# ashual/scene_generation

Hardware: AMD Instinct MI355X
Metric: images/sec G+D step, 128x128 <=8-obj scene graphs (higher is better)
Workload: dtype f32

## Files before the change

### scene_generation_amd/csrc/common.h

```cpp
#pragma once
#include <hip/hip_runtime.h>
#include <stdint.h>
#include <stdio.h>
#include <atomic>
#include "../../include/sg2im_hip.h"

#define SG_WAVE 64

void sg_set_error(const char* fmt, ...);
int sg_check_indices_if_enabled(const int64_t* idx, int64_t n, int64_t lo, int64_t hi, const char* what, hipStream_t s);

#define SG_ARG_CHECK(cond, ...)                 \
  do {                                          \
    if (!(cond)) {                              \
      sg_set_error(__VA_ARGS__);                \
      return -1;                                \
    }                                           \
  } while (0)

#define SG_LAUNCH_CHECK(name)                                               \
  do {                                                                      \
    hipError_t e__ = hipGetLastError();                                     \
    if (e__ != hipSuccess) {                                                \
      sg_set_error("%s: launch failed: %s", name, hipGetErrorString(e__)); \
      return (int)e__;                                                      \
    }                                                                       \
  } while (0)

enum SgOpt {
  SG_OPT_TILE,
  SG_OPT_T128_MIN,
  SG_OPT_TILE3,
  SG_OPT_TILE3_MIN,
  SG_OPT_SPLIT_TARGET,
  SG_OPT_SPLIT_KMIN,
  SG_OPT_SPLITS,
  SG_OPT_FIXEDTAP,
  SG_OPT_WINO_WT,
  SG_OPT_W24_SMALL,
  SG_OPT_W24_S,
  SG_OPT_W24_PMIN,
  SG_OPT_WINO_ADJOINT,
  SG_OPT_WINO24,
  SG_OPT_LINEAR_NSUB,
  SG_OPT_LINEAR_SKINNY,
  SG_OPT_WGRAD_ROWSUM,
  SG_OPT_LAYOUT_REG,
  SG_OPT_LAYOUT_DSPLIT,
  SG_OPT_BN_BLOCKS,
  SG_OPT_INSTNORM_REG,
  SG_OPT_WGRAD_XCD,
  SG_OPT_WINO_REUSE,
  SG_OPT_WINO_FOLD_CELLS,
  SG_OPT_WINO_PIPE,
  SG_OPT_CHECK_INDICES,
  SG_OPT_LAST_BLOCK,
  SG_OPT_WINO_GEMM_TILE,
  SG_OPT_WINO43,
  SG_OPT_GCONV_FUSED_GATHER,
  SG_OPT_W24_GEMM_TILE,
  SG_OPT_WINO_IN_FUSE,
  SG_OPT_W43_NSUB,
  SG_OPT_W43_KFOLD,
  SG_OPT_WAVE_PRIO,
  SG_OPT_PAR_XCD_CHUNK,
  SG_OPT_W43_TAIL_SPLIT,
  SG_OPT_TAIL_SMAX,
  SG_OPT_TAIL_KTMIN,
  SG_OPT_W43_WGRAD_TILE,
  SG_OPT_PAR_SPLIT,
  SG_OPT_TAIL_CAPTURE,
  SG_OPT_WGRAD_PADDED,
  SG_OPT_COUNT
};
extern std::atomic<int> g_sg_opt[SG_OPT_COUNT];
static inline int sg_opt(int id) { return g_sg_opt[id].load(std::memory_order_relaxed); }
extern FILE* g_sg_launch_log;

enum {
  SG_K_IGEMM_BASE = 0, SG_K_IGEMM_COUNT = 48,
  SG_K_LINEAR = 48, SG_K_LAYOUT_FWD, SG_K_LAYOUT_BWD, SG_K_INSTNORM, SG_K_BATCHNORM, SG_K_ADAM, SG_K_SEGSUM,
  SG_K_CROP, SG_K_OTHER,
  SG_K_WINO_GEMM_128, SG_K_WINO_GEMM_64, SG_K_WINO_XFORM,
  SG_K_HEAD,
  SG_K_INSTNORM_BWD,
  SG_K_WINO24_GEMM,
  SG_K_WINO43_GEMM,
  SG_K_LAYOUT_TEST_PLANES,
  SG_K_DEPROCESS,
  SG_K_LAYOUT_RGB,
  SG_K_KMEANS_ASSIGN, SG_K_KMEANS_UPDATE, SG_K_KMEANS_RELOCATE, SG_K_KMEANS_PP,
  SG_K_SCENEGRAPH_CENTERS, SG_K_SCENEGRAPH_DERIVE, SG_K_SCENEGRAPH_AGREE,
  SG_K_MAXPOOL3S2, SG_K_ADD_RELU, SG_K_BN_FOLD, SG_K_SGD, SG_K_CLASSIFY_STATS,
  SG_K_RECT_CONV_T64, SG_K_RECT_CONV_T32, SG_K_RECT_CONV_T64W, SG_K_RECT_REDUCE, SG_K_INCEPTION_POOL, SG_K_RESIZE_BILINEAR,
  SG_K_SOFTMAX_ROWS, SG_K_INCEPTION_SCORE,
  SG_K_FID_MOMENTS,
  SG_K_WIDE_CONV, SG_K_LPIPS_INPUT, SG_K_LPIPS_LAYER,
  SG_K_FEAT_POLY, SG_K_FEAT_MANIFOLD,
  SG_K_PIL_RESIZE,
  SG_K_FIDINF_GRAMS, SG_K_FIDINF_TERMS,
  SG_K_COUNT
};
static inline int sg_igemm_kind(int family, int KS, int tile) {
  const int k = KS == 1 ? 0 : (KS == 3 ? 1 : (KS == 4 ? 2 : 3));
  return SG_K_IGEMM_BASE + family * 16 + k * 4 + tile;
}
extern int g_sg_prof_on;
void sg_prof_begin(int kind, hipStream_t s);
void sg_prof_end(int kind, hipStream_t s, double flops, double bytes);

struct SgProfScope {
  int kind; hipStream_t s; double flops, bytes; bool on;
  SgProfScope(int k, hipStream_t st, double f, double b) : kind(k), s(st), flops(f), bytes(b), on(g_sg_prof_on != 0) {
    if (on) sg_prof_begin(kind, s);
  }
  ~SgProfScope() { if (on) sg_prof_end(kind, s, flops, bytes); }
};

struct FastDiv {
  unsigned m, s, d;
  FastDiv() : m(0), s(0), d(1) {}
  explicit FastDiv(unsigned dd) : m(0), s(0), d(dd) {
    if (dd > 1) {
      unsigned sh = 0;
      while ((1u << sh) < dd) ++sh;
      m = (unsigned)((((uint64_t)1) << (31 + sh)) / dd + 1);
      s = sh - 1;
    }
  }
  __device__ __forceinline__ unsigned div(unsigned n) const { return d == 1 ? n : (__umulhi(n, m) >> s); }
};

static inline int sg_cdiv(int64_t a, int64_t b) { return (int)((a + b - 1) / b); }

__device__ __forceinline__ float sg_apply_act(float v, int act, float slope) {
  switch (act) {
    case SG_ACT_RELU: return v > 0.f ? v : 0.f;
    case SG_ACT_LEAKY: return v > 0.f ? v : v * slope;
    case SG_ACT_TANH: return tanhf(v);
    case SG_ACT_SIGMOID: return 1.f / (1.f + expf(-v));
    default: return v;
  }
}

__device__ __forceinline__ float sg_wave_sum(float v) {
#pragma unroll
  for (int o = 32; o > 0; o >>= 1) v += __shfl_xor(v, o, 64);
  return v;
}

__device__ __forceinline__ float sg_sum_strided(const float* __restrict__ p, size_t stride, int S) {
  float v = 0.f;
  for (int z0 = 0; z0 < S; z0 += 8) {
    float t[8];
#pragma unroll
    for (int e = 0; e < 8; ++e) t[e] = z0 + e < S ? p[(size_t)(z0 + e) * stride] : 0.f;
#pragma unroll
    for (int e = 0; e < 8; ++e)
      if (z0 + e < S) v += t[e];
  }
  return v;
}

__device__ __forceinline__ void sg_publish(float* p, float v) { __hip_atomic_store(p, v, __ATOMIC_RELAXED, __HIP_MEMORY_SCOPE_AGENT); }
__device__ __forceinline__ float sg_consume(const float* p) {
  return __hip_atomic_load(const_cast<float*>(p), __ATOMIC_RELAXED, __HIP_MEMORY_SCOPE_AGENT);
}
__device__ __forceinline__ bool sg_arrive_last(int* counter, int narrive, int* flag) {
  asm volatile("s_waitcnt vmcnt(0)" ::: "memory");
  __syncthreads();
  if (threadIdx.x == 0 && threadIdx.y == 0 && threadIdx.z == 0) {
    const int t = __hip_atomic_fetch_add(counter, 1, __ATOMIC_RELAXED, __HIP_MEMORY_SCOPE_AGENT);
    const int last = t == narrive - 1;
    if (last) __hip_atomic_store(counter, 0, __ATOMIC_RELAXED, __HIP_MEMORY_SCOPE_AGENT);
    *flag = last;
  }
  __syncthreads();
  return *flag != 0;
}
int* sg_counter_alloc(hipStream_t s, int n = 1, bool always = false, int family = 1);
float* sg_tail_scratch(hipStream_t s, size_t bytes);

__device__ __forceinline__ float sg_block_sum(float v, float* red) {
  const int lane = threadIdx.x & 63, wid = threadIdx.x >> 6, nw = (blockDim.x + 63) >> 6;
  v = sg_wave_sum(v);
  __syncthreads();
  if (lane == 0) red[wid] = v;
  __syncthreads();
  float t = 0.f;
  for (int i = 0; i < nw; ++i) t += red[i];
  return t;
}
```

### scene_generation_amd/csrc/igemm.hip

```cpp
#include "igemm_core.h"

namespace sgk {
thread_local double t_alg_bytes = 0.0;
std::mutex g_tab_mu;
std::map<TabKey, TabEntry> g_tabs;
size_t g_tab_bytes = 0;
}

namespace {
int check_desc(const sgConvDesc* d, const char* who) {
  SG_ARG_CHECK(d != nullptr, "%s: null desc", who);
  SG_ARG_CHECK(d->KS == 1 || d->KS == 3 || d->KS == 4 || d->KS == 7, "%s: kernel size %d unsupported", who, d->KS);
  SG_ARG_CHECK(d->stride == 1 || d->stride == 2, "%s: stride %d unsupported", who, d->stride);
  SG_ARG_CHECK(d->upsample == 1 || d->upsample == 2, "%s: upsample %d unsupported", who, d->upsample);
  SG_ARG_CHECK(d->N > 0 && d->C1 > 0 && d->C2 >= 0 && d->Cout > 0 && d->H > 0 && d->W > 0 && d->OH > 0 && d->OW > 0,
               "%s: non-positive dimension", who);
  SG_ARG_CHECK(!d->pad_reflect || d->pad < d->H * d->upsample, "%s: reflect pad too large", who);
  const double lim = SG_MAX_ELEMS;
  SG_ARG_CHECK((double)d->N * (d->C1 + d->C2) * d->H * d->W <= lim && (double)d->N * d->Cout * d->OH * d->OW <= lim &&
                   (double)d->N * (d->C1 + d->C2) * (d->H * d->upsample + 2.0 * d->pad) *
                           (d->W * d->upsample + 2.0 * d->pad) <= lim &&
                   (double)d->Cout * (d->C1 + d->C2) * d->KS * d->KS <= lim,
               "%s: a tensor has more than %.0f elements (32-bit offsets%s)", who, lim,
               SG_BUFLOAD ? ", buffer-load range masking" : "");
// ... 1119 lines not shown
      if (rb >= 0 && ca >= 0) v += acc[rb * PW + ca];
      if (rb >= 0 && cb >= 0) v += acc[rb * PW + cb];
      so[a * W + b] = v;
    }
  }
  __syncthreads();
  float* dstg = gx + ((size_t)n * C + c0) * HW;
  for (int i = threadIdx.x * 4; i < 64 * HW; i += 1024) {
    const int ch = i / HW, px = i - ch * HW;
    const float* sp = stage + ch * (HW + 1) + px;
    *reinterpret_cast<float4*>(dstg + i) = make_float4(sp[0], sp[1], sp[2], sp[3]);
  }
}

template <int TPT>
__global__ void __launch_bounds__(256) w43_output_in_kernel(const float* __restrict__ Mx, const float* __restrict__ bias,
                                                           const float* __restrict__ skip, float* __restrict__ ypre,
                                                           float* __restrict__ out, float* __restrict__ mean_o,
                                                           float* __restrict__ rstd_o, int N, int M, int H, int W, float eps, int act,
                                                           float slope) {
  extern __shared__ __attribute__((aligned(16))) float lds[];
  const int HW = H * W, TH = H / 4, TW = W / 4, NT = TH * TW, pitch = HW + 1;
  const int n = blockIdx.y, c0 = blockIdx.x * 64, c = threadIdx.x & 63, g = threadIdx.x >> 6, m = c0 + c;
  float* sa = lds;
  float* sb = lds + 64 * pitch;
  float* red = lds + 128 * pitch;
  const float b = bias ? bias[m] : 0.f;
  const size_t ld = (size_t)36 * M;
  float o[TPT][4][4];
  float s = 0.f;
#pragma unroll
  for (int k = 0; k < TPT; ++k) {
    const int t = g + 4 * k;
    if (t < NT) {
      const float* src = Mx + ((size_t)n * NT + t) * ld + m;
      float q[6][6];
#pragma unroll
      for (int i = 0; i < 36; ++i) q[i / 6][i % 6] = src[(size_t)i * M];
      w43_output_xform(q, o[k]);
#pragma unroll
      for (int a = 0; a < 4; ++a)
#pragma unroll
        for (int e = 0; e < 4; ++e) { o[k][a][e] += b; s += o[k][a][e]; }
    }
  }
  red[g * 64 + c] = s;
  __syncthreads();
  const float mean = (((red[c] + red[64 + c]) + red[128 + c]) + red[192 + c]) / (float)HW;
  __syncthreads();
  float qv = 0.f;
#pragma unroll
  for (int k = 0; k < TPT; ++k)
    if (g + 4 * k < NT) {
#pragma unroll
      for (int a = 0; a < 4; ++a)
#pragma unroll
        for (int e = 0; e < 4; ++e) { const float dlt = o[k][a][e] - mean; qv += dlt * dlt; }
    }
  red[g * 64 + c] = qv;
  __syncthreads();
  const float rstd = 1.f / sqrtf((((red[c] + red[64 + c]) + red[128 + c]) + red[192 + c]) / (float)HW + eps);
  if (g == 0) { mean_o[(size_t)n * M + m] = mean; rstd_o[(size_t)n * M + m] = rstd; }
#pragma unroll
  for (int k = 0; k < TPT; ++k) {
    const int t = g + 4 * k;
    if (t < NT) {
      const int ti = t / TW, tj = t - ti * TW;
#pragma unroll
      for (int a = 0; a < 4; ++a)
#pragma unroll
        for (int e = 0; e < 4; ++e) {
          const int px = (4 * ti + a) * W + 4 * tj + e;
          sa[c * pitch + px] = o[k][a][e];
          sb[c * pitch + px] = sg_apply_act((o[k][a][e] - mean) * rstd, act, slope);
        }
    }
  }
  __syncthreads();
  const size_t base = ((size_t)n * M + c0) * HW;
  for (int i = threadIdx.x * 4; i < 64 * HW; i += 1024) {
    const int ch = i / HW, px = i - ch * HW;
    const float* pa = sa + ch * pitch + px;
    const float* pb = sb + ch * pitch + px;
    *reinterpret_cast<float4*>(ypre + base + i) = make_float4(pa[0], pa[1], pa[2], pa[3]);
    float4 v = make_float4(pb[0], pb[1], pb[2], pb[3]);
    if (skip) {
      const float4 k4 = *reinterpret_cast<const float4*>(skip + base + i);
      v.x += k4.x; v.y += k4.y; v.z += k4.z; v.w += k4.w;
    }
    *reinterpret_cast<float4*>(out + base + i) = v;
  }
}

__global__ void __launch_bounds__(256) w43_gy_in_kernel(const float* __restrict__ gout, const float* __restrict__ ypre,
                                                       const float* __restrict__ mean_i, const float* __restrict__ rstd_i,
                                                       float* __restrict__ gconv, float* __restrict__ Ytp, float* __restrict__ gb_part,
                                                       int N, int M, int H, int W, int act, float slope) {
  extern __shared__ __attribute__((aligned(16))) float lds[];
  const int HW = H * W, pitch = HW + 1, TH = H / 4, TW = W / 4, NT = TH * TW;
  const int n = blockIdx.y, c0 = blockIdx.x * 64, tid = threadIdx.x, c = tid & 63, g = tid >> 6;
  float* pg = lds;
  float* px = lds + 64 * pitch;
  float* red = lds + 128 * pitch;
  const size_t base = ((size_t)n * M + c0) * HW;
  w43_stage_planes(gout + base, pg, HW, tid);
  w43_stage_planes(ypre + base, px, HW, tid);
  __syncthreads();
  const float mean = mean_i[(size_t)n * M + c0 + c], rstd = rstd_i[(size_t)n * M + c0 + c];
  float* gc = pg + c * pitch;
  const float* xc = px + c * pitch;
  float s1 = 0.f, s2 = 0.f;
  for (int t = g; t < NT; t += 4) {
    const int ti = t / TW, tj = t - ti * TW;
#pragma unroll
    for (int a = 0; a < 4; ++a)
#pragma unroll
      for (int e = 0; e < 4; ++e) {
        const int p = (4 * ti + a) * W + 4 * tj + e;
        const float z = (xc[p] - mean) * rstd;
        const float gp = gc[p] * act_grad_from_pre_w(z, act, slope);
        s1 += gp; s2 += gp * z;
      }
  }
  red[g * 64 + c] = s1;
  red[256 + g * 64 + c] = s2;
  __syncthreads();
  const float inv = 1.f / (float)HW;
  const float m1 = (((red[c] + red[64 + c]) + red[128 + c]) + red[192 + c]) * inv;
  const float m2 = (((red[256 + c] + red[320 + c]) + red[384 + c]) + red[448 + c]) * inv;
  const size_t P = (size_t)N * NT;
  float sb = 0.f;
  for (int t = g; t < NT; t += 4) {
    const int ti = t / TW, tj = t - ti * TW;
    float gt[4][4];
#pragma unroll
    for (int a = 0; a < 4; ++a)
#pragma unroll
      for (int e = 0; e < 4; ++e) {
        const int p = (4 * ti + a) * W + 4 * tj + e;
        const float z = (xc[p] - mean) * rstd;
        const float gp = gc[p] * act_grad_from_pre_w(z, act, slope);
        gt[a][e] = rstd * (gp - m1 - z * m2);
        gc[p] = gt[a][e];
        sb += gt[a][e];
      }
    float yt[6][6];
    w43_gy_xform(gt, yt);
    const size_t p = (size_t)n * NT + t;
#pragma unroll
    for (int i = 0; i < 6; ++i)
#pragma unroll
      for (int j = 0; j < 6; ++j) Ytp[((size_t)(i * 6 + j) * P + p) * M + c0 + c] = yt[i][j];
  }
  red[512 + g * 64 + c] = sb;
  __syncthreads();
  if (gb_part != nullptr && g == 0)
    gb_part[(size_t)n * M + c0 + c] = ((red[512 + c] + red[576 + c]) + red[640 + c]) + red[704 + c];
  for (int i = tid * 4; i < 64 * HW; i += 1024) {
    const int ch = i / HW, q = i - ch * HW;
    const float* sp = pg + ch * pitch + q;
    *reinterpret_cast<float4*>(gconv + base + i) = make_float4(sp[0], sp[1], sp[2], sp[3]);
  }
}

__global__ void w43_bias_sum_kernel(const float* __restrict__ part, float* __restrict__ gb, int N, int M) {
  const int m = blockIdx.x * blockDim.x + threadIdx.x;
  if (m >= M) return;
  float v = 0.f;
  for (int n0 = 0; n0 < N; n0 += 8) {
    float t[8];
#pragma unroll
    for (int e = 0; e < 8; ++e) t[e] = n0 + e < N ? part[(size_t)(n0 + e) * M + m] : 0.f;
#pragma unroll
    for (int e = 0; e < 8; ++e) v += t[e];
  }
  gb[m] = v;
}

__global__ void w43_wgrad_output_kernel(const float* __restrict__ T, float* __restrict__ gw, int M, int C) {
  const size_t idx = (size_t)blockIdx.x * blockDim.x + threadIdx.x;
  if (idx >= (size_t)M * C) return;
  const int c = (int)(idx % C);
  const size_t m = idx / C;
  const float* src = T + m * 36 * C + c;
  float q[6][6];
#pragma unroll
  for (int i = 0; i < 36; ++i) q[i / 6][i % 6] = src[(size_t)i * C];
  float o[3][3];
  w43_wgrad_xform(q, o);
  float* dst = gw + idx * 9;
#pragma unroll
  for (int a = 0; a < 3; ++a)
#pragma unroll
    for (int b = 0; b < 3; ++b) dst[a * 3 + b] = o[a][b];
}

void w43_launch_weight(const float* w, float* U, int R, int Cc, hipStream_t s) {
  SgProfScope xf(SG_K_WINO_XFORM, s, 0, 4.0 * 45.0 * (double)R * Cc);
  hipLaunchKernelGGL(w43_weight_kernel, dim3((R / 32) * (Cc / 32)), dim3(256), 0, s, w, U, R, Cc);
}
void w43_launch_input(const float* x, float* V, int N, int C, int H, int W, size_t P, hipStream_t s) {
  SgProfScope xf(SG_K_WINO_XFORM, s, 0, 4.0 * ((double)N * C * H * W + 36.0 * (double)P * C));
  const size_t lds = (size_t)64 * (H * W + 1) * sizeof(float);
  wino_lds_attr(&w43_input_kernel, lds);
  hipLaunchKernelGGL(w43_input_kernel, dim3(C / 64, N), dim3(256), lds, s, x, V, N, C, H, W);
}
void w43_launch_gy(const float* gy, float* Ytp, int N, int M, int H, int W, size_t P, hipStream_t s) {
  SgProfScope xf(SG_K_WINO_XFORM, s, 0, 4.0 * ((double)N * M * H * W + 36.0 * (double)P * M));
  const size_t lds = (size_t)64 * (H * W + 1) * sizeof(float);
  wino_lds_attr(&w43_gy_kernel, lds);
  hipLaunchKernelGGL(w43_gy_kernel, dim3(M / 64, N), dim3(256), lds, s, gy, Ytp, N, M, H, W);
}
void w43_launch_fold(const float* G, float* gx, int N, int C, int H, int W, size_t P, hipStream_t s) {
  SgProfScope xf(SG_K_WINO_XFORM, s, 0, 4.0 * (36.0 * (double)P * C + (double)N * C * H * W));
  const size_t lds = (size_t)64 * ((H + 2) * (W + 2) + 1 + H * W + 1) * sizeof(float);
  wino_lds_attr(&w43_fold_kernel, lds);
  hipLaunchKernelGGL(w43_fold_kernel, dim3(C / 64, N), dim3(256), lds, s, G, gx, N, C, H, W);
}
}

__device__ __forceinline__ void w24_bt(const float (&d)[5], float (&o)[5]) {
  o[0] = -2.f * d[0] - d[1] + 2.f * d[2] + d[3];
  o[1] = 2.f * d[1] + 3.f * d[2] + d[3];
  o[2] = -2.f * d[1] + d[2] + d[3];
  o[3] = d[3] - d[1];
  o[4] = -2.f * d[1] - d[2] + 2.f * d[3] + d[4];
}
__device__ __forceinline__ void w24_g(const float (&g)[4], float (&o)[5]) {
  o[0] = -0.5f * g[0];
  o[1] = (g[0] + g[1] + g[2] + g[3]) * (1.f / 6.f);
  o[2] = (g[0] - g[1] + g[2] - g[3]) * 0.5f;
  o[3] = (-g[0] + 2.f * g[1] - 4.f * g[2] + 8.f * g[3]) * (1.f / 6.f);
  o[4] = g[3];
}
__device__ __forceinline__ void w24_at(const float (&m)[5], float (&o)[2]) {
  o[0] = m[0] + m[1] + m[2] + m[3];
  o[1] = m[1] - m[2] - 2.f * m[3] + m[4];
}
__device__ __forceinline__ void w24_a(const float (&y)[2], float (&o)[5]) {
  o[0] = y[0]; o[1] = y[0] + y[1]; o[2] = y[0] - y[1]; o[3] = y[0] - 2.f * y[1]; o[4] = y[1];
}
__device__ __forceinline__ void w24_gt(const float (&t)[5], float (&o)[4]) {
  o[0] = -0.5f * t[0] + (t[1] - t[3]) * (1.f / 6.f) + 0.5f * t[2];
  o[1] = (t[1] + 2.f * t[3]) * (1.f / 6.f) - 0.5f * t[2];
  o[2] = (t[1] - 4.f * t[3]) * (1.f / 6.f) + 0.5f * t[2];
  o[3] = (t[1] + 8.f * t[3]) * (1.f / 6.f) - 0.5f * t[2] + t[4];
}

template <int KMAJ>
__global__ void w24_input_kernel(const float* __restrict__ x, float* __restrict__ V, int N, int C, int H, int W, int TH, int TW,
                                 int off, size_t Pstride, int Pc, int S) {
  const size_t P = (size_t)N * TH * TW, total = Pstride * C;
  const size_t idx = (size_t)blockIdx.x * blockDim.x + threadIdx.x;
  if (idx >= total) return;
  const size_t p = KMAJ ? idx % Pstride : idx / C;
  const int c = (int)(KMAJ ? idx / Pstride : idx % C);
  float d[5][5];
  if (p < P) {
    const int n = (int)(p / (TH * TW)), r = (int)(p - (size_t)n * TH * TW), ti = r / TW, tj = r - ti * TW;
    const float* xp = x + ((size_t)n * C + c) * H * W;
#pragma unroll
    for (int a = 0; a < 5; ++a) {
      const int ih = 2 * ti + off + a;
      const bool rok = (unsigned)ih < (unsigned)H;
#pragma unroll
      for (int b = 0; b < 5; ++b) {
        const int iw = 2 * tj + off + b;
        const bool ok = rok && (unsigned)iw < (unsigned)W;
        d[a][b] = ok ? xp[ih * W + iw] : 0.f;
      }
    }
  } else {
#pragma unroll
    for (int a = 0; a < 5; ++a)
#pragma unroll
      for (int b = 0; b < 5; ++b) d[a][b] = 0.f;
  }
  float t[5][5];
#pragma unroll
  for (int j = 0; j < 5; ++j) {
    const float col[5] = {d[0][j], d[1][j], d[2][j], d[3][j], d[4][j]};
    float o[5];
    w24_bt(col, o);
#pragma unroll
    for (int i = 0; i < 5; ++i) t[i][j] = o[i];
  }
#pragma unroll
  for (int i = 0; i < 5; ++i) {
    float o[5];
    w24_bt(t[i], o);
#pragma unroll
    for (int j = 0; j < 5; ++j) {
      const size_t xi = (size_t)(i * 5 + j);
      if (KMAJ) {
        const size_t sidx = p / (size_t)Pc, pc = p - sidx * (size_t)Pc;
        V[((xi * S + sidx) * C + c) * (size_t)Pc + pc] = o[j];
      } else {
        V[(xi * Pstride + p) * C + c] = o[j];
      }
    }
  }
}

__global__ void __launch_bounds__(256) w24_input_small_kernel(const float* __restrict__ x, float* __restrict__ V, int N, int C, int H,
                                                             int W, int TH, int TW, int off, size_t Pstride, int rows_per,
                                                             int pitch) {
  extern __shared__ __attribute__((aligned(16))) float pl[];
  const int HW = H * W;
  const int n = blockIdx.y, c0 = blockIdx.x * 64, tid = threadIdx.x;
  const int tr0 = (int)blockIdx.z * rows_per, tr1 = min(TH, tr0 + rows_per);
  const int lane = tid & 63, g = tid >> 6;
  const int rlo = max(0, 2 * tr0 + off), rhi = min(H, 2 * (tr1 - 1) + off + 5);
  {
    const int cnt = (rhi - rlo) * W;
    const float* src = x + ((size_t)n * C + c0) * HW + rlo * W;
    for (int ch = g; ch < 64; ch += 4)
      for (int e = lane; e < cnt; e += 64) pl[ch * pitch + e] = src[(size_t)ch * HW + e];
  }
  __syncthreads();
  const float* pc = pl + lane * pitch - rlo * W;
  const size_t P = (size_t)N * TH * TW;
  for (int t = tr0 * TW + g; t < tr1 * TW; t += 4) {
    const int ti = t / TW, tj = t - ti * TW;
    float d[5][5];
#pragma unroll
    for (int a = 0; a < 5; ++a) {
      const int ih = 2 * ti + off + a;
      const bool rok = (unsigned)ih < (unsigned)H;
#pragma unroll
      for (int b = 0; b < 5; ++b) {
        const int iw = 2 * tj + off + b;
        const bool ok = rok && (unsigned)iw < (unsigned)W;
        d[a][b] = ok ? pc[ih * W + iw] : 0.f;
      }
    }
    float tt[5][5];
#pragma unroll
    for (int j = 0; j < 5; ++j) {
      const float col[5] = {d[0][j], d[1][j], d[2][j], d[3][j], d[4][j]};
      float o[5];
      w24_bt(col, o);
#pragma unroll
      for (int i = 0; i < 5; ++i) tt[i][j] = o[i];
    }
    const size_t p = (size_t)n * TH * TW + t;
#pragma unroll
    for (int i = 0; i < 5; ++i) {
      float o[5];
      w24_bt(tt[i], o);
#pragma unroll
      for (int j = 0; j < 5; ++j) V[((size_t)(i * 5 + j) * Pstride + p) * C + c0 + lane] = o[j];
    }
  }
  if (n == 0 && blockIdx.z == 0)
    for (size_t p = P + g; p < Pstride; p += 4)
      for (int xi = 0; xi < 25; ++xi) V[((size_t)xi * Pstride + p) * C + c0 + lane] = 0.f;
}
inline bool w24_small_geom(int N, int C, int H, int W, int TH, int* rows_per_out, int* pitch_out) {
  int rows_per = (int)(((long)(C / 64) * N * TH + 2047) / 2048);
  if (rows_per < 1) rows_per = 1;
  const int nrows = std::min(H, 2 * rows_per + 3);
  const int pitch = (nrows * W) | 1;
  if ((size_t)64 * pitch * sizeof(float) > 64 * 1024) return false;
  *rows_per_out = rows_per;
  *pitch_out = pitch;
  return true;
}
void w24_input_pc(int kernel, const float* x, float* V, int N, int C, int H, int W, int TH, int TW, int off, size_t Pstride,
                  hipStream_t s) {
  const int HW = H * W;
  SgProfScope xf(SG_K_WINO_XFORM, s, 0, 4.0 * ((double)N * C * HW + 25.0 * (double)Pstride * C));
  if (kernel == SG_WK_IN_LDS) {
    int rows_per = 0, pitch = 0;
    w24_small_geom(N, C, H, W, TH, &rows_per, &pitch);
    const size_t lds = (size_t)64 * pitch * sizeof(float);
    wino_lds_attr(&w24_input_small_kernel, lds);
    hipLaunchKernelGGL(w24_input_small_kernel, dim3(C / 64, N, sg_cdiv(TH, rows_per)), dim3(256), lds, s, x, V, N, C, H, W, TH, TW, off,
                       Pstride, rows_per, pitch);
    return;
  }
  hipLaunchKernelGGL(w24_input_kernel<0>, dim3(sg_cdiv(Pstride * C, 256)), dim3(256), 0, s, x, V, N, C, H, W, TH, TW, off, Pstride, 0, 1);
}

__global__ void w24_weight_kernel(const float* __restrict__ w, float* __restrict__ U, int R, int Cc, int mode) {
  const size_t idx = (size_t)blockIdx.x * blockDim.x + threadIdx.x;
  if (idx >= (size_t)R * Cc) return;
  const int c = (int)(idx % Cc), r = (int)(idx / Cc);
  const float* g = w + (mode ? ((size_t)c * R + r) : ((size_t)r * Cc + c)) * 16;
  float k[4][4];
#pragma unroll
  for (int i = 0; i < 16; ++i) k[i >> 2][i & 3] = mode ? g[15 - i] : g[i];
  float t[5][4];
#pragma unroll
  for (int j = 0; j < 4; ++j) {
    const float col[4] = {k[0][j], k[1][j], k[2][j], k[3][j]};
    float o[5];
    w24_g(col, o);
#pragma unroll
    for (int i = 0; i < 5; ++i) t[i][j] = o[i];
  }
#pragma unroll
  for (int i = 0; i < 5; ++i) {
    float o[5];
    w24_g(t[i], o);
#pragma unroll
    for (int j = 0; j < 5; ++j) U[((size_t)(i * 5 + j) * R + r) * Cc + c] = o[j];
  }
}

__global__ void w24_output_kernel(const float* __restrict__ Mx, const float* __restrict__ bias, float* __restrict__ y, int N,
                                  int M, int OH, int OW, int TH, int TW, size_t Pstride, int act, float slope) {
  const size_t P = (size_t)N * TH * TW;
  const size_t idx = (size_t)blockIdx.x * blockDim.x + threadIdx.x;
  if (idx >= P * M) return;
  const size_t p = idx % P;
  const int m = (int)(idx / P);
  const float* src = Mx + (size_t)m * 25 * Pstride + p;
  float q[5][5];
#pragma unroll
  for (int i = 0; i < 25; ++i) q[i / 5][i % 5] = src[(size_t)i * Pstride];
  float sres[2][5];
#pragma unroll
  for (int j = 0; j < 5; ++j) {
    const float col[5] = {q[0][j], q[1][j], q[2][j], q[3][j], q[4][j]};
    float o[2];
    w24_at(col, o);
    sres[0][j] = o[0]; sres[1][j] = o[1];
  }
  const float b = bias ? bias[m] : 0.f;
  const int n = (int)(p / (TH * TW)), r = (int)(p - (size_t)n * TH * TW), ti = r / TW, tj = r - ti * TW;
  float* o = y + (((size_t)n * M + m) * OH + 2 * ti) * OW + 2 * tj;
#pragma unroll
  for (int a = 0; a < 2; ++a) {
    float v[2];
    w24_at(sres[a], v);
    if (2 * ti + a < OH) {
      o[a * OW] = sg_apply_act(v[0] + b, act, slope);
      if (2 * tj + 1 < OW) o[a * OW + 1] = sg_apply_act(v[1] + b, act, slope);
    }
  }
}

__global__ void w24_gy_kernel(const float* __restrict__ gy, float* __restrict__ Yt, int N, int M, int OH, int OW, int TH, int TW,
                              size_t Pstride, int Pc, int S) {
  const size_t P = (size_t)N * TH * TW;
  const size_t idx = (size_t)blockIdx.x * blockDim.x + threadIdx.x;
  if (idx >= Pstride * M) return;
  const size_t p = idx % Pstride;
  const int m = (int)(idx / Pstride);
  float y2[2][2] = {{0.f, 0.f}, {0.f, 0.f}};
  if (p < P) {
    const int n = (int)(p / (TH * TW)), r = (int)(p - (size_t)n * TH * TW), ti = r / TW, tj = r - ti * TW;
    const float* g = gy + (((size_t)n * M + m) * OH + 2 * ti) * OW + 2 * tj;
#pragma unroll
    for (int a = 0; a < 2; ++a)
#pragma unroll
      for (int b = 0; b < 2; ++b)
        if (2 * ti + a < OH && 2 * tj + b < OW) y2[a][b] = g[a * OW + b];
  }
  float t[5][2];
#pragma unroll
  for (int j = 0; j < 2; ++j) {
    const float col[2] = {y2[0][j], y2[1][j]};
    float o[5];
    w24_a(col, o);
#pragma unroll
    for (int i = 0; i < 5; ++i) t[i][j] = o[i];
  }
  const size_t sidx = p / (size_t)Pc, pc = p - sidx * (size_t)Pc;
#pragma unroll
  for (int i = 0; i < 5; ++i) {
    float o[5];
    w24_a(t[i], o);
#pragma unroll
    for (int j = 0; j < 5; ++j) Yt[(((size_t)(i * 5 + j) * S + sidx) * M + m) * (size_t)Pc + pc] = o[j];
  }
}

__global__ void w24_wgrad_output_kernel(const float* __restrict__ T, float* __restrict__ gw, int M, int C, int S) {
  const size_t idx = (size_t)blockIdx.x * blockDim.x + threadIdx.x;
  if (idx >= (size_t)M * C) return;
  const int c = (int)(idx % C), m = (int)(idx / C);
  const float* src = T + (size_t)m * 25 * S * C + c;
  float q[5][5];
#pragma unroll
  for (int i = 0; i < 25; ++i) q[i / 5][i % 5] = 0.f;
  for (int z = 0; z < S; ++z) {
    float t[25];
#pragma unroll
    for (int i = 0; i < 25; ++i) t[i] = src[((size_t)i * S + z) * C];
#pragma unroll
    for (int i = 0; i < 25; ++i) q[i / 5][i % 5] += t[i];
  }
  float t[4][5];
#pragma unroll
  for (int j = 0; j < 5; ++j) {
    const float col[5] = {q[0][j], q[1][j], q[2][j], q[3][j], q[4][j]};
    float o[4];
    w24_gt(col, o);
#pragma unroll
    for (int i = 0; i < 4; ++i) t[i][j] = o[i];
  }
  float* dst = gw + ((size_t)m * C + c) * 16;
#pragma unroll
  for (int i = 0; i < 4; ++i) {
    float o[4];
    w24_gt(t[i], o);
    *reinterpret_cast<float4*>(dst + i * 4) = make_float4(o[0], o[1], o[2], o[3]);
  }
}

struct W24Plan { int TH, TW, THd, TWd; size_t P, Ps, Pd, Pds; int S, Pc; };
bool w24_plan(const sgConvDesc* d, W24Plan* pl) {
  if (!d || d->KS != 4 || d->stride != 1 || d->C2 != 0 || d->upsample != 1 || d->pad_reflect || d->pad < 0 || d->pad > 3) return false;
  if (d->C1 % 128 != 0 || d->Cout % 128 != 0 || d->OH < 2 || d->OW < 2) return false;
  if (d->OH != d->H + 2 * d->pad - 3 || d->OW != d->W + 2 * d->pad - 3) return false;
  W24Plan p;
  p.TH = (d->OH + 1) / 2; p.TW = (d->OW + 1) / 2;
  p.THd = (d->H + 1) / 2; p.TWd = (d->W + 1) / 2;
  p.P = (size_t)d->N * p.TH * p.TW; p.Pd = (size_t)d->N * p.THd * p.TWd;
  p.Ps = (p.P + 127) / 128 * 128; p.Pds = (p.Pd + 127) / 128 * 128;
  const long t = 25L * (d->Cout / 128) * (d->C1 / 128);
  int S = (int)((400 + t - 1) / t);
  if (sg_opt(SG_OPT_W24_S) > 0) S = sg_opt(SG_OPT_W24_S);
  const int maxS = (int)(p.P / 256) > 0 ? (int)(p.P / 256) : 1;
  if (S > maxS) S = maxS;
  if (S < 1) S = 1;
  p.Pc = (int)(((p.P + S - 1) / S + 31) / 32 * 32);
  p.S = (int)((p.P + p.Pc - 1) / p.Pc);
  const double cm = d->C1 > d->Cout ? d->C1 : d->Cout;
  const double pm = (double)(p.Ps > p.Pds ? p.Ps : p.Pds) + 32.0 * p.S;
  if (!(25.0 * pm * cm < 2147483647.0 && 25.0 * (double)d->C1 * d->Cout < 2147483647.0)) return false;
  if (p.P < (size_t)sg_opt(SG_OPT_W24_PMIN)) return false;
  if (pl) *pl = p;
  return true;
}

int wino_class(const sgConvDesc* d) {
  if (!wino_ok(d)) return SG_WF_UNSUPPORTED;
  if (!(sg_opt(SG_OPT_WINO_ADJOINT) && d->pad_reflect && d->upsample == 1 && d->H * d->W <= 256 && (d->H * d->W) % 4 == 0 &&
        d->C1 % 64 == 0 && d->Cout % 64 == 0))
    return SG_WF_F23_GENERIC;
  if (!sg_opt(SG_OPT_WINO43) || d->H % 4 != 0 || d->W % 4 != 0) return SG_WF_F23_ADJOINT;
  const double P = (double)d->N * (d->H / 4) * (d->W / 4), Cmax = d->C1 > d->Cout ? d->C1 : d->Cout;
  return ((long)P % 64 == 0 && 36.0 * P * Cmax < SG_MAX_ELEMS && 36.0 * d->C1 * d->Cout < SG_MAX_ELEMS) ? SG_WF_F43 : SG_WF_F23_ADJOINT;
}
size_t wino_tiles(const sgConvDesc* d, int t) { return (size_t)d->N * (d->H * d->upsample / t) * (d->W * d->upsample / t); }
size_t wino_dgrad_tiles(const sgConvDesc* d) {
  const size_t T = (size_t)wino_tile(d);
  const size_t P = d->pad_reflect ? (size_t)d->N * (d->H * d->upsample / 2 + 1) * (d->W * d->upsample / 2 + 1) : wino_tiles(d, 2);
  return (P + T - 1) / T * T;
}
size_t wino_ut_floats(const sgConvDesc* d, int cls) {
  return cls == SG_WF_F43 ? (size_t)36 * d->C1 * d->Cout : cls == SG_WF_F23_ADJOINT ? (size_t)16 * d->C1 * d->Cout : 0;
}
size_t wino_kept_floats(const sgConvDesc* d, int cls, int ch) {
  if (!sg_opt(SG_OPT_WINO_REUSE) || cls < SG_WF_F23_ADJOINT) return 0;
  return cls == SG_WF_F43 ? 36 * wino_tiles(d, 4) * ch : 16 * wino_tiles(d, 2) * ch;
}
bool wino_in_ok(const sgConvDesc* d, int cls) {
  return sg_opt(SG_OPT_WINO_IN_FUSE) && cls == SG_WF_F43 && (d->H / 4) * (d->W / 4) <= 16 && sg_opt(SG_OPT_WINO_REUSE);
}

bool wino_weight_lds(int R, int Cc, bool w16) { return sg_opt(SG_OPT_WINO_WT) && R % 32 == 0 && Cc % 32 == 0 && w16; }
bool wino_input_small(int C, int H, int W, int ush, bool x16) {
  return ush == 0 && H * W <= 256 && (H * W) % 4 == 0 && C % 64 == 0 && x16;
}
bool w24_input_small(int N, int C, int H, int W, int TH) {
  int rows_per, pitch;
  return sg_opt(SG_OPT_W24_SMALL) && H * W >= 144 && W <= 64 && C % 64 == 0 && w24_small_geom(N, C, H, W, TH, &rows_per, &pitch);
}
void wino_set_gemm(sgWinoPlan* p, int bm, int bn, int nsub, int kfold, int pipe) {
  p->bm = bm; p->bn = bn; p->nsub = nsub; p->kfold = kfold; p->pipe = pipe;
}
void wino_gemm_sel(sgWinoPlan* p, int NB, int M, int cols, int K) {
  const int t = NB == 16 ? sg_opt(SG_OPT_WINO_GEMM_TILE) : sg_opt(SG_OPT_W24_GEMM_TILE);
  const bool fits = M % 64 == 0 && cols % 128 == 0 && K % 32 == 0;
  if (t == 1 && fits) wino_set_gemm(p, 64, 128, 2, 0, 0);
  else if (t == 2 && fits) wino_set_gemm(p, 64, 64, 2, 0, 0);
  else wino_set_gemm(p, 128, 128, 2, 0, sg_opt(SG_OPT_WINO_PIPE) == 2 ? 2 : 1);
}
bool w43_deep() { return sg_opt(SG_OPT_W43_NSUB) != 1; }
void w43_gemm_sel(sgWinoPlan* p, int K) {
  const int kf = sg_opt(SG_OPT_W43_KFOLD);
  wino_set_gemm(p, 64, 64, w43_deep() ? 2 : 1, (K > 256 || (K > 128 && kf == 128)) ? kf : 0, 0);
}
void w43_wgrad_sel(sgWinoPlan* p, int M, int C, int P) {
  const int wt = sg_opt(SG_OPT_W43_WGRAD_TILE);
  if (wt == 1 && M % 128 == 0 && C % 128 == 0 && P % 32 == 0) wino_set_gemm(p, 128, 128, 2, 0, 0);
  else if (wt == 2 && C % 128 == 0 && P % 32 == 0) wino_set_gemm(p, 64, 128, 2, 0, 0);
  else wino_set_gemm(p, 64, 64, w43_deep() ? 2 : 1, 0, 0);
}

#define WP_CHECK(cond, msg) do { if (!(cond)) { *err = (msg); return -1; } } while (0)
int wino_launch_plan(const sgConvDesc* d, int entry, int align_mask, int saved_mask, sgWinoPlan* out, const char** err) {
  const bool x16 = align_mask & SG_WA_X, w16 = align_mask & SG_WA_W, y16 = align_mask & SG_WA_Y, gy16 = align_mask & SG_WA_GY,
             gx16 = align_mask & SG_WA_GX, gw16 = align_mask & SG_WA_GW;
  const bool ut = saved_mask & SG_WS_UT, v = saved_mask & SG_WS_V, ytp = saved_mask & SG_WS_YTP;
  sgWinoPlan p = {};
  if (entry >= SG_WINO24_FWD) {
    W24Plan w;
    WP_CHECK(w24_plan(d, &w), "unsupported desc");
    WP_CHECK(saved_mask == 0, "F(2x2,4x4) takes no saved operands");
    p.form = SG_WF_F24;
    p.P = (int)w.P; p.Ps = (int)w.Ps; p.Pd = (int)w.Pd; p.Pds = (int)w.Pds;
    p.TH = w.TH; p.TW = w.TW; p.THd = w.THd; p.TWd = w.TWd; p.S = w.S; p.Pc = w.Pc;
    if (entry == SG_WINO24_FWD) {
      p.in_kernel = w24_input_small(d->N, d->C1, d->H, d->W, w.TH) ? SG_WK_IN_LDS : SG_WK_IN_GENERAL;
      p.wt_kernel = SG_WK_WT_PLAIN;
      wino_gemm_sel(&p, 25, d->Cout, (int)w.Ps, d->C1);
    } else if (entry == SG_WINO24_DGRAD) {
      p.in_kernel = w24_input_small(d->N, d->Cout, d->OH, d->OW, w.THd) ? SG_WK_IN_LDS : SG_WK_IN_GENERAL;
      p.wt_kernel = SG_WK_WT_PLAIN;
      wino_gemm_sel(&p, 25, d->C1, (int)w.Pds, d->Cout);
    } else {
      WP_CHECK(gw16, "gw must be 16-byte aligned");
      p.in_kernel = SG_WK_IN_GENERAL;
      p.wgrad_src = SG_WSRC_REBUILT;
      wino_gemm_sel(&p, 25 * w.S, d->Cout, d->C1, w.Pc);
    }
    *out = p;
    return 0;
  }
  const int cls = wino_class(d);
  const bool fused = entry == SG_WINO_FWD_INSTNORM || entry == SG_WINO_DGRAD_INSTNORM;
  WP_CHECK(cls != SG_WF_UNSUPPORTED && (!fused || wino_in_ok(d, cls)), "unsupported desc");
  const int LH = d->H * d->upsample, LW = d->W * d->upsample, refl = d->pad_reflect;
  if (cls == SG_WF_F43) {
    p.form = SG_WF_F43;
    p.P = p.Ps = p.Pd = p.Pds = (int)wino_tiles(d, 4);
    if (entry == SG_WINO_FWD || entry == SG_WINO_FWD_INSTNORM) {
      WP_CHECK(x16 && w16 && y16, fused ? "operands must be 16-byte aligned" : "F(4x4,3x3) shapes need 16-byte aligned x / y / w");
      WP_CHECK(!ytp, "the forward takes no ytp_save");
      p.in_kernel = SG_WK_IN_LDS; p.wt_kernel = SG_WK_WT_LDS;
      w43_gemm_sel(&p, d->C1);
      if (fused) p.norm_tiles = (d->H / 4) * (d->W / 4) <= 4 ? 1 : 4;
    } else if (entry == SG_WINO_DGRAD || entry == SG_WINO_DGRAD_INSTNORM) {
      WP_CHECK(gy16 && gx16 && w16, fused ? "operands must be 16-byte aligned" : "F(4x4,3x3) shapes need 16-byte aligned gy / gx / w");
      WP_CHECK(!v, "the data gradient takes no v_save");
      p.in_kernel = SG_WK_IN_LDS; p.wt_kernel = ut ? SG_WK_NONE : SG_WK_WT_LDS; p.fold_kernel = SG_WK_FOLD_F43;
      w43_gemm_sel(&p, d->Cout);
    } else {
      WP_CHECK(x16 && gy16, "F(4x4,3x3) shapes need 16-byte aligned x / gy");
      WP_CHECK(!ut, "the weight gradient takes no ut_save");
      const bool saved = v && ytp;
      p.wgrad_src = saved ? SG_WSRC_SAVED : SG_WSRC_REBUILT;
      p.in_kernel = saved ? SG_WK_NONE : SG_WK_IN_LDS;
      w43_wgrad_sel(&p, d->Cout, d->C1, p.P);
    }
    *out = p;
    return 0;
  }
  p.P = p.Ps = (int)wino_tiles(d, 2);
  p.Pd = d->N * (LH / 2 + (refl ? 1 : 0)) * (LW / 2 + (refl ? 1 : 0));
  p.Pds = (int)wino_dgrad_tiles(d);
  if (entry == SG_WINO_FWD) {
    WP_CHECK(!ytp, "the forward takes no ytp_save");
    WP_CHECK(!v || wino_kept_floats(d, cls, d->C1) > 0, "v_save given but unused by this desc");
    WP_CHECK(!ut || wino_ut_floats(d, cls) > 0, "ut_save given but unused by this desc");
    const bool lds = wino_weight_lds(d->Cout, d->C1, w16);
    WP_CHECK(!ut || lds, "the transposed filter transform needs the LDS weight kernel");
    p.form = SG_WF_F23_GENERIC;
    p.wt_kernel = lds ? SG_WK_WT_LDS : SG_WK_WT_PLAIN;
    p.in_kernel = wino_input_small(d->C1, LH, LW, d->upsample == 2 ? 1 : 0, x16) ? SG_WK_IN_LDS : SG_WK_IN_GENERAL;
    wino_gemm_sel(&p, 16, d->Cout, p.P, d->C1);
  } else if (entry == SG_WINO_DGRAD) {
    WP_CHECK(!v, "the data gradient takes no v_save");
    const int M = d->C1, K = d->Cout;
    if (cls == SG_WF_F23_ADJOINT && gy16 && gx16) {
      p.form = SG_WF_F23_ADJOINT;
      p.Pd = p.Pds = p.P;
      p.in_kernel = SG_WK_IN_LDS;
      p.wt_kernel = ut ? SG_WK_NONE : (wino_weight_lds(M, K, w16) ? SG_WK_WT_LDS : SG_WK_WT_PLAIN);
      p.fold_kernel = sg_opt(SG_OPT_WINO_FOLD_CELLS) ? SG_WK_FOLD_CELLS : SG_WK_FOLD_WALK;
      wino_gemm_sel(&p, 16, p.P, M, K);
    } else {
      WP_CHECK(!ytp, "ytp_save given but this desc does not run the adjoint form");
      p.form = SG_WF_F23_GENERIC;
      p.wt_kernel = wino_weight_lds(M, K, w16) ? SG_WK_WT_LDS : SG_WK_WT_PLAIN;
      p.in_kernel = wino_input_small(K, LH, LW, 0, gy16) ? SG_WK_IN_LDS : SG_WK_IN_GENERAL;
      p.fold_kernel = (!refl && d->upsample == 1) ? SG_WK_NONE : SG_WK_FOLD_PAD_UPSAMPLE;
// ... 574 lines not shown
```

### scene_generation_amd/csrc/runtime.hip

```cpp
#include "common.h"
#include <stdarg.h>
#include <mutex>
#include <vector>
#include <stdlib.h>
#include <string.h>
#include <ctype.h>

static thread_local char t_err[512] = "ok";

void sg_set_error(const char* fmt, ...) {
  va_list ap;
  va_start(ap, fmt);
  vsnprintf(t_err, sizeof(t_err), fmt, ap);
  va_end(ap);
}

extern "C" const char* sg_last_error_string(void) { return t_err; }
extern "C" int sg_version(void) { return 100; }

int g_sg_prof_on = 0;

std::atomic<int> g_sg_opt[SG_OPT_COUNT];
FILE* g_sg_launch_log = nullptr;
namespace {
struct OptDef { const char* name; int def; };
const OptDef kOpts[SG_OPT_COUNT] = {
    {"tile", -1}, {"t128_min", 384}, {"tile3", 1}, {"tile3_min", 768}, {"split_target", 1536}, {"split_kmin", 2048}, {"splits", -1}, {"fixedtap", 1}, {"wino_wt", 1},
    {"w24_small", 1}, {"w24_s", -1}, {"w24_pmin", 256}, {"wino_adjoint", 1}, {"wino24", 1}, {"linear_nsub", 2},
    {"linear_skinny", 2048}, {"wgrad_rowsum", 1}, {"layout_reg", 1}, {"layout_dsplit", 1}, {"bn_blocks", 4096},
    {"instnorm_reg", 2}, {"wgrad_xcd", 1}, {"wino_reuse", 1}, {"wino_fold_cells", 1}, {"wino_pipe", 2},
    {"check_indices", 0}, {"last_block", 0}, {"wino_gemm_tile", 0}, {"wino43", 1}, {"gconv_fused_gather", 1}, {"w24_gemm_tile", 2}, {"wino_in_fuse", 1}, {"w43_nsub", 1}, {"w43_kfold", 256}, {"wave_prio", 0}, {"par_xcd_chunk", 16}, {"w43_tail_split", 2}, {"tail_smax", 4}, {"tail_ktmin", 8}, {"w43_wgrad_tile", 0}, {"par_split", 1}, {"tail_capture", 1}, {"wgrad_padded", 1}};
struct OptInit {
  OptInit() {
    for (int i = 0; i < SG_OPT_COUNT; ++i) {
      char env[64] = "SG_";
      size_t n = 3;
      for (const char* c = kOpts[i].name; *c && n + 1 < sizeof(env); ++c) env[n++] = (char)toupper((unsigned char)*c);
      env[n] = 0;
      const char* e = getenv(env);
      g_sg_opt[i].store((e && *e) ? atoi(e) : kOpts[i].def, std::memory_order_relaxed);
    }
    const char* lf = getenv("SG_LAUNCH_LOG");
    if (lf && *lf) g_sg_launch_log = fopen(lf, "a");
  }
} g_opt_init;
int opt_index(const char* key) {
  if (!key) return -1;
  for (int i = 0; i < SG_OPT_COUNT; ++i)
    if (strcmp(key, kOpts[i].name) == 0) return i;
  return -1;
}
}

extern "C" int sg_num_options(void) { return SG_OPT_COUNT; }
extern "C" const char* sg_option_name(int i) { return (i >= 0 && i < SG_OPT_COUNT) ? kOpts[i].name : nullptr; }
extern "C" int sg_option_default(int i) { return (i >= 0 && i < SG_OPT_COUNT) ? kOpts[i].def : 0; }
extern "C" int sg_get_option(const char* key, int* value) {
  const int i = opt_index(key);
  if (i < 0 || !value) { sg_set_error("sg_get_option: unknown option '%s'", key ? key : "(null)"); return -1; }
  *value = sg_opt(i);
  return 0;
}
extern "C" int sg_set_option(const char* key, int value) {
  const int i = opt_index(key);
  if (i < 0) { sg_set_error("sg_set_option: unknown option '%s'", key ? key : "(null)"); return -1; }
  g_sg_opt[i].store(value, std::memory_order_relaxed);
  return 0;
}

namespace {
constexpr int CNT_RING = 65536, CNT_CAPTURED = 262144, CNT_DEVICES = 16;
std::mutex g_cnt_mu;
int* g_cnt_pool[CNT_DEVICES] = {};
unsigned g_cnt_ring[CNT_DEVICES] = {};
int g_cnt_cap[CNT_DEVICES] = {};
}

int* sg_counter_alloc(hipStream_t s, int n, bool always, int family) {
  if ((!always && !(sg_opt(SG_OPT_LAST_BLOCK) & family)) || n < 1 || n > 4096) return nullptr;
  int dev = 0;
  if (hipGetDevice(&dev) != hipSuccess || dev < 0 || dev >= CNT_DEVICES) return nullptr;
  hipStreamCaptureStatus cap = hipStreamCaptureStatusNone;
  const bool capturing = hipStreamIsCapturing(s, &cap) == hipSuccess && cap != hipStreamCaptureStatusNone;
  std::lock_guard<std::mutex> lk(g_cnt_mu);
  if (!g_cnt_pool[dev]) {
    if (capturing) return nullptr;
    int* p = nullptr;
    const size_t bytes = (size_t)(CNT_RING + CNT_CAPTURED) * sizeof(int);
    if (hipMalloc((void**)&p, bytes) != hipSuccess) return nullptr;
    if (hipMemset(p, 0, bytes) != hipSuccess) { hipFree(p); return nullptr; }
    g_cnt_pool[dev] = p;
  }
  if (capturing) {
    if (g_cnt_cap[dev] + n > CNT_CAPTURED) return nullptr;
    int* r = g_cnt_pool[dev] + CNT_RING + g_cnt_cap[dev];
    g_cnt_cap[dev] += n;
    return r;
  }
  unsigned at = g_cnt_ring[dev];
  if (at + (unsigned)n > (unsigned)CNT_RING) at = 0;
  g_cnt_ring[dev] = at + (unsigned)n;
  return g_cnt_pool[dev] + at;
}

namespace {
struct TailScratch { int dev; hipStream_t s; float* p; size_t bytes; };
std::vector<TailScratch> g_tail;
}

namespace {
struct TailCap { float* p; size_t bytes; };
TailCap g_tail_cap[CNT_DEVICES] = {};
void tail_cap_reserve(int dev, size_t bytes) {
  if (dev < 0 || dev >= CNT_DEVICES || g_tail_cap[dev].bytes >= bytes) return;
  float* q = nullptr;
  if (hipMalloc((void**)&q, bytes) != hipSuccess) return;
  g_tail_cap[dev].p = q; g_tail_cap[dev].bytes = bytes;
}
}

float* sg_tail_scratch(hipStream_t s, size_t bytes) {
  int dev = 0;
  if (hipGetDevice(&dev) != hipSuccess) return nullptr;
  hipStreamCaptureStatus cap = hipStreamCaptureStatusNone;
  const bool capturing = hipStreamIsCapturing(s, &cap) == hipSuccess && cap != hipStreamCaptureStatusNone;
  std::lock_guard<std::mutex> lk(g_cnt_mu);
  if (capturing)
    return (sg_opt(SG_OPT_TAIL_CAPTURE) && dev >= 0 && dev < CNT_DEVICES && g_tail_cap[dev].bytes >= bytes) ? g_tail_cap[dev].p : nullptr;
  tail_cap_reserve(dev, bytes);
  for (auto& t : g_tail)
    if (t.dev == dev && t.s == s) {
      if (t.bytes >= bytes) return t.p;
      float* q = nullptr;
      if (hipMalloc((void**)&q, bytes) != hipSuccess) return nullptr;
      t.p = q; t.bytes = bytes;
      return q;
    }
  float* q = nullptr;
  if (hipMalloc((void**)&q, bytes) != hipSuccess) return nullptr;
  g_tail.push_back(TailScratch{dev, s, q, bytes});
  return q;
}

namespace {
struct Rec { int kind; hipEvent_t e0, e1; double flops, bytes; };
std::mutex g_mu;
std::vector<Rec> g_recs;
std::vector<hipEvent_t> g_free;
hipEvent_t g_open[SG_K_COUNT];
double g_ms[SG_K_COUNT], g_flops[SG_K_COUNT], g_bytes[SG_K_COUNT];
int64_t g_cnt[SG_K_COUNT];
const char* kTail[SG_K_COUNT - SG_K_IGEMM_COUNT] = {"linear", "layout_fwd", "layout_bwd", "instnorm", "batchnorm", "adam",
                                                    "segsum", "crop", "other", "wino_bgemm_t128", "wino_bgemm_t64",
                                                    "wino_transforms", "head_conv", "instnorm_bwd", "wino24_bgemm_t128", "wino43_bgemm_t64",
                                                    "layout_test_planes", "deprocess", "layout_rgb", "kmeans_assign", "kmeans_update",
                                                    "kmeans_relocate", "kmeans_pp", "scenegraph_centers", "scenegraph_derive",
                                                    "scenegraph_agree", "maxpool3s2", "add_relu", "bn_fold", "sgd", "classify_stats",
                                                    "rect_conv_t64", "rect_conv_t32", "rect_conv_t64x128", "rect_reduce", "inception_pool",
                                                    "resize_bilinear", "softmax_rows", "inception_score", "fid_moments", "wide_conv_t64",
                                                    "lpips_input", "lpips_layer", "feat_poly", "feat_manifold", "pil_resize",
                                                    "fidinf_grams", "fidinf_terms"};
char g_names[SG_K_COUNT][32];
bool g_names_init = false;
void init_names() {
  if (g_names_init) return;
  const char* fam[3] = {"kn0", "kn1", "nk"};
  const int ks[4] = {1, 3, 4, 7};
  const char* tl[4] = {"128", "64", "32", "64x128"};
  for (int f = 0; f < 3; ++f)
    for (int k = 0; k < 4; ++k)
      for (int t = 0; t < 4; ++t)
        snprintf(g_names[f * 16 + k * 4 + t], 32, "igemm_%s_k%d_t%s", fam[f], ks[k], tl[t]);
  for (int i = SG_K_IGEMM_COUNT; i < SG_K_COUNT; ++i) snprintf(g_names[i], 32, "%s", kTail[i - SG_K_IGEMM_COUNT]);
  g_names_init = true;
}

hipEvent_t get_event() {
  if (!g_free.empty()) { hipEvent_t e = g_free.back(); g_free.pop_back(); return e; }
  hipEvent_t e;
  hipEventCreate(&e);
  return e;
}

void drain() {
  for (auto& r : g_recs) {
    hipEventSynchronize(r.e1);
    float ms = 0.f;
    hipEventElapsedTime(&ms, r.e0, r.e1);
    g_ms[r.kind] += ms; g_flops[r.kind] += r.flops; g_bytes[r.kind] += r.bytes; g_cnt[r.kind] += 1;
    g_free.push_back(r.e0); g_free.push_back(r.e1);
  }
  g_recs.clear();
}
}

void sg_prof_begin(int kind, hipStream_t s) {
  std::lock_guard<std::mutex> lk(g_mu);
  hipEvent_t e = get_event();
  hipEventRecord(e, s);
  g_open[kind] = e;
}

void sg_prof_end(int kind, hipStream_t s, double flops, double bytes) {
  std::lock_guard<std::mutex> lk(g_mu);
  hipEvent_t e = get_event();
  hipEventRecord(e, s);
  g_recs.push_back(Rec{kind, g_open[kind], e, flops, bytes});
  if (g_recs.size() > 8192) drain();
}

extern "C" int sg_prof_enable(int on) { g_sg_prof_on = on; return 0; }
extern "C" int sg_prof_reset(void) {
  std::lock_guard<std::mutex> lk(g_mu);
  drain();
  for (int i = 0; i < SG_K_COUNT; ++i) { g_ms[i] = g_flops[i] = g_bytes[i] = 0; g_cnt[i] = 0; }
  return 0;
}
extern "C" int sg_prof_num_kinds(void) { return SG_K_COUNT; }
extern "C" const char* sg_prof_kind_name(int kind) {
  init_names();
  return (kind >= 0 && kind < SG_K_COUNT) ? g_names[kind] : "?";
}
extern "C" int sg_prof_read(int kind, double* total_ms, int64_t* launches, double* flops, double* bytes) {
  if (kind < 0 || kind >= SG_K_COUNT) { sg_set_error("sg_prof_read: bad kind %d", kind); return -1; }
  std::lock_guard<std::mutex> lk(g_mu);
  drain();
  if (total_ms) *total_ms = g_ms[kind];
  if (launches) *launches = g_cnt[kind];
  if (flops) *flops = g_flops[kind];
  if (bytes) *bytes = g_bytes[kind];
  return 0;
}
```

Before: 1143.

## Stage Winograd F(2,4) input tiles in LDS with vectorized loads and adaptive geometry

Rewrites the LDS-staged Winograd 2x4 input transform so it loads input planes with float4 vector loads batched eight per thread, picks rows-per-block and wave count from a new geometry helper, and spreads zero-padding writes across all blocks instead of one. It also sends general (non-small) cases with W<=64 and aligned input through the staged path under a new default-on option. The aim is to cut global-load inefficiency and the serialized padding tail in the input transform. The risks are more LDS per block and larger blocks, up to 768 threads, which may lower occupancy, and extra index arithmetic in the vector path.

```diff
diff --git a/scene_generation_amd/csrc/common.h b/scene_generation_amd/csrc/common.h
--- a/scene_generation_amd/csrc/common.h
+++ b/scene_generation_amd/csrc/common.h
@@ -71,6 +71,7 @@
   SG_OPT_PAR_SPLIT,
   SG_OPT_TAIL_CAPTURE,
   SG_OPT_WGRAD_PADDED,
+  SG_OPT_W24_STAGE,
   SG_OPT_COUNT
 };
 extern std::atomic<int> g_sg_opt[SG_OPT_COUNT];
diff --git a/scene_generation_amd/csrc/igemm.hip b/scene_generation_amd/csrc/igemm.hip
--- a/scene_generation_amd/csrc/igemm.hip
+++ b/scene_generation_amd/csrc/igemm.hip
@@ -1445,25 +1445,62 @@
   }
 }
 
-__global__ void __launch_bounds__(256) w24_input_small_kernel(const float* __restrict__ x, float* __restrict__ V, int N, int C, int H,
+template <bool VEC>
+__global__ void __launch_bounds__(768) w24_input_small_kernel(const float* __restrict__ x, float* __restrict__ V, int N, int C, int H,
                                                              int W, int TH, int TW, int off, size_t Pstride, int rows_per,
                                                              int pitch) {
   extern __shared__ __attribute__((aligned(16))) float pl[];
   const int HW = H * W;
-  const int n = blockIdx.y, c0 = blockIdx.x * 64, tid = threadIdx.x;
-  const int tr0 = (int)blockIdx.z * rows_per, tr1 = min(TH, tr0 + rows_per);
-  const int lane = tid & 63, g = tid >> 6;
+  const int bx = blockIdx.x, n = blockIdx.y, bz = blockIdx.z;
+  const int c0 = bx * 64, tid = threadIdx.x, nthr = blockDim.x;
+  const int tr0 = bz * rows_per, tr1 = min(TH, tr0 + rows_per);
+  const int lane = tid & 63, g = tid >> 6, nw = nthr >> 6;
   const int rlo = max(0, 2 * tr0 + off), rhi = min(H, 2 * (tr1 - 1) + off + 5);
   {
-    const int cnt = (rhi - rlo) * W;
-    const float* src = x + ((size_t)n * C + c0) * HW + rlo * W;
-    for (int ch = g; ch < 64; ch += 4)
-      for (int e = lane; e < cnt; e += 64) pl[ch * pitch + e] = src[(size_t)ch * HW + e];
+    const int cnt = (rhi - rlo) * W, s0 = rlo * W;
+    const float* blk = x + ((size_t)n * C + c0) * HW;
+    if (VEC) {
+      const int nv = (cnt >> 2) + 2, total = cnt > 0 ? 64 * nv : 0;
+      for (int i0 = tid; i0 < total; i0 += 8 * nthr) {
+        float4 v[8];
+#pragma unroll
+        for (int e = 0; e < 8; ++e) {
+          const int i = i0 + e * nthr, ch = i / nv, s = ch * HW + s0, a = (s & ~3) + 4 * (i - ch * nv);
+          if (i < total && a < s + cnt) v[e] = *reinterpret_cast<const float4*>(blk + a);
+        }
+#pragma unroll
+        for (int e = 0; e < 8; ++e) {
+          const int i = i0 + e * nthr, ch = i / nv, s = ch * HW + s0, a = (s & ~3) + 4 * (i - ch * nv);
+          if (i < total && a < s + cnt) {
+            float* d = pl + ch * pitch + (a - s);
+            const float q[4] = {v[e].x, v[e].y, v[e].z, v[e].w};
+#pragma unroll
+            for (int j = 0; j < 4; ++j)
+              if ((unsigned)(a - s + j) < (unsigned)cnt) d[j] = q[j];
+          }
+        }
+      }
+    } else {
+      const int total = cnt > 0 ? 64 * cnt : 0;
+      for (int i0 = tid; i0 < total; i0 += 8 * nthr) {
+        float v[8];
+#pragma unroll
+        for (int e = 0; e < 8; ++e) {
+          const int i = i0 + e * nthr, ch = i / cnt;
+          if (i < total) v[e] = blk[(size_t)ch * HW + s0 + (i - ch * cnt)];
+        }
+#pragma unroll
+        for (int e = 0; e < 8; ++e) {
+          const int i = i0 + e * nthr, ch = i / cnt;
+          if (i < total) pl[ch * pitch + (i - ch * cnt)] = v[e];
+        }
+      }
+    }
   }
   __syncthreads();
   const float* pc = pl + lane * pitch - rlo * W;
   const size_t P = (size_t)N * TH * TW;
-  for (int t = tr0 * TW + g; t < tr1 * TW; t += 4) {
+  for (int t = tr0 * TW + g; t < tr1 * TW; t += nw) {
     const int ti = t / TW, tj = t - ti * TW;
     float d[5][5];
 #pragma unroll
@@ -1495,9 +1532,8 @@
       for (int j = 0; j < 5; ++j) V[((size_t)(i * 5 + j) * Pstride + p) * C + c0 + lane] = o[j];
     }
   }
-  if (n == 0 && blockIdx.z == 0)
-    for (size_t p = P + g; p < Pstride; p += 4)
-      for (int xi = 0; xi < 25; ++xi) V[((size_t)xi * Pstride + p) * C + c0 + lane] = 0.f;
+  for (size_t p = P + (size_t)n * gridDim.z + bz; p < Pstride; p += (size_t)N * gridDim.z)
+    for (int xi = g; xi < 25; xi += nw) V[((size_t)xi * Pstride + p) * C + c0 + lane] = 0.f;
 }
 inline bool w24_small_geom(int N, int C, int H, int W, int TH, int* rows_per_out, int* pitch_out) {
   int rows_per = (int)(((long)(C / 64) * N * TH + 2047) / 2048);
@@ -1509,17 +1545,41 @@
   *pitch_out = pitch;
   return true;
 }
+inline void w24_stage_geom(int N, int C, int H, int W, int TH, int TW, int* rows_per_out, int* pitch_out, int* waves_out) {
+  const long groups = (long)(C / 64) * N;
+  int splits = (int)std::min<long>(TH, (256 + groups - 1) / groups);
+  int rows_per = (TH + splits - 1) / splits;
+  while (rows_per > 1 && (groups * ((TH + rows_per - 1) / rows_per) < 256 ||
+                          (size_t)64 * ((std::min(H, 2 * rows_per + 3) * W) | 1) * sizeof(float) > 96 * 1024)) {
+    ++splits;
+    rows_per = (TH + splits - 1) / splits;
+  }
+  *rows_per_out = rows_per;
+  *pitch_out = (std::min(H, 2 * rows_per + 3) * W) | 1;
+  const int tiles = rows_per * TW, rounds = (tiles + 11) / 12;
+  *waves_out = (tiles + rounds - 1) / rounds;
+}
+inline bool w24_general_staged(const float* x, int N, int C, int H, int W, int TH) {
+  int rows_per, pitch;
+  return sg_opt(SG_OPT_W24_STAGE) && W <= 64 && C % 64 == 0 && ((uintptr_t)x & 15) == 0 &&
+         w24_small_geom(N, C, H, W, TH, &rows_per, &pitch);
+}
 void w24_input_pc(int kernel, const float* x, float* V, int N, int C, int H, int W, int TH, int TW, int off, size_t Pstride,
                   hipStream_t s) {
   const int HW = H * W;
   SgProfScope xf(SG_K_WINO_XFORM, s, 0, 4.0 * ((double)N * C * HW + 25.0 * (double)Pstride * C));
-  if (kernel == SG_WK_IN_LDS) {
-    int rows_per = 0, pitch = 0;
-    w24_small_geom(N, C, H, W, TH, &rows_per, &pitch);
+  if (kernel == SG_WK_IN_LDS || w24_general_staged(x, N, C, H, W, TH)) {
+    int rows_per = 0, pitch = 0, waves = 0;
+    w24_stage_geom(N, C, H, W, TH, TW, &rows_per, &pitch, &waves);
     const size_t lds = (size_t)64 * pitch * sizeof(float);
-    wino_lds_attr(&w24_input_small_kernel, lds);
-    hipLaunchKernelGGL(w24_input_small_kernel, dim3(C / 64, N, sg_cdiv(TH, rows_per)), dim3(256), lds, s, x, V, N, C, H, W, TH, TW, off,
-                       Pstride, rows_per, pitch);
+    const dim3 grid(C / 64, N, sg_cdiv(TH, rows_per)), block(64 * waves);
+    if (((uintptr_t)x & 15) == 0) {
+      wino_lds_attr(&w24_input_small_kernel<true>, lds);
+      hipLaunchKernelGGL(w24_input_small_kernel<true>, grid, block, lds, s, x, V, N, C, H, W, TH, TW, off, Pstride, rows_per, pitch);
+    } else {
+      wino_lds_attr(&w24_input_small_kernel<false>, lds);
+      hipLaunchKernelGGL(w24_input_small_kernel<false>, grid, block, lds, s, x, V, N, C, H, W, TH, TW, off, Pstride, rows_per, pitch);
+    }
     return;
   }
   hipLaunchKernelGGL(w24_input_kernel<0>, dim3(sg_cdiv(Pstride * C, 256)), dim3(256), 0, s, x, V, N, C, H, W, TH, TW, off, Pstride, 0, 1);
diff --git a/scene_generation_amd/csrc/runtime.hip b/scene_generation_amd/csrc/runtime.hip
--- a/scene_generation_amd/csrc/runtime.hip
+++ b/scene_generation_amd/csrc/runtime.hip
@@ -29,7 +29,7 @@
     {"w24_small", 1}, {"w24_s", -1}, {"w24_pmin", 256}, {"wino_adjoint", 1}, {"wino24", 1}, {"linear_nsub", 2},
     {"linear_skinny", 2048}, {"wgrad_rowsum", 1}, {"layout_reg", 1}, {"layout_dsplit", 1}, {"bn_blocks", 4096},
     {"instnorm_reg", 2}, {"wgrad_xcd", 1}, {"wino_reuse", 1}, {"wino_fold_cells", 1}, {"wino_pipe", 2},
-    {"check_indices", 0}, {"last_block", 0}, {"wino_gemm_tile", 0}, {"wino43", 1}, {"gconv_fused_gather", 1}, {"w24_gemm_tile", 2}, {"wino_in_fuse", 1}, {"w43_nsub", 1}, {"w43_kfold", 256}, {"wave_prio", 0}, {"par_xcd_chunk", 16}, {"w43_tail_split", 2}, {"tail_smax", 4}, {"tail_ktmin", 8}, {"w43_wgrad_tile", 0}, {"par_split", 1}, {"tail_capture", 1}, {"wgrad_padded", 1}};
+    {"check_indices", 0}, {"last_block", 0}, {"wino_gemm_tile", 0}, {"wino43", 1}, {"gconv_fused_gather", 1}, {"w24_gemm_tile", 2}, {"wino_in_fuse", 1}, {"w43_nsub", 1}, {"w43_kfold", 256}, {"wave_prio", 0}, {"par_xcd_chunk", 16}, {"w43_tail_split", 2}, {"tail_smax", 4}, {"tail_ktmin", 8}, {"w43_wgrad_tile", 0}, {"par_split", 1}, {"tail_capture", 1}, {"wgrad_padded", 1}, {"w24_stage", 1}};
 struct OptInit {
   OptInit() {
     for (int i = 0; i < SG_OPT_COUNT; ++i) {
```

Result: no change. 1148 (median of 6 runs) (+0.5%).
